# mkocabas/EpipolarPose

Measured on AMD Instinct MI355X. Metric: images/sec (4-view 256x256, ResNet-50) at 1/2/4/8 MI355X; MPJPE vs ref, higher is better.
Workload: dtype bf16; 1 GPU; configs[1]: ResNet-50 Integral-pose, 4-view 256x256 synthetic, batch=32/GPU, fully-supervised SmoothL1 loss; global_batch=32, joints=17, depth_res=64, optimizer=adam, parallelism=dp1, launch=eager, streams=2, deterministic=True

## Files before the change

### epipolarpose_amd/csrc/head_gemm.hip

```cpp
#include "common.h"
#include "bn_affine.h"
#include <algorithm>
#include <cstdlib>
#include <mutex>
#include <type_traits>
#include <unordered_map>
#include <utility>
#include <vector>

namespace epi {

typedef __bf16 bf16x8 __attribute__((ext_vector_type(8)));
typedef float f32x16 __attribute__((ext_vector_type(16)));

constexpr int GBK = 64;

template <int TM_, int WM_, int WN_, int MIN_WAVES_, int NSTAGE_, bool STAGGER_ = false> struct GemmCfg {
    static constexpr int TM = TM_, WM = WM_, WN = WN_, NW = WM_ * WN_, THREADS = 64 * NW, MIN_WAVES = MIN_WAVES_, NSTAGE = NSTAGE_;
    static constexpr bool STAGGER = STAGGER_;
    static constexpr int BM = WM_ * TM_ * 32, BN = WN_ * 64;
    static constexpr int A_BYTES = BM * 128, B_BYTES = BN * 128, STAGE_BYTES = A_BYTES + B_BYTES;
    static constexpr int AP = BM / 8 / NW, BP = BN / 8 / NW;
    static constexpr bool EARLY = NW == 4 && NSTAGE_ == 2;
    static_assert(AP >= 1 && BP >= 1 && BM % (8 * NW) == 0 && BN % (8 * NW) == 0, "whole pieces per wave");
// ... 1099 lines not shown
    if (OUT_F32) {
        *reinterpret_cast<float4v*>(reinterpret_cast<float*>(p.C) + orow * p.ldc + n) = a;
    } else {
        if (p.addend) {
            const uint2 r = *reinterpret_cast<const uint2*>(p.addend + orow * p.ldc + n);
            a.x = bf16_to_f32(f32_to_bf16(a.x)) + __uint_as_float(r.x << 16); a.y = bf16_to_f32(f32_to_bf16(a.y)) + __uint_as_float(r.x & 0xffff0000u);
            a.z = bf16_to_f32(f32_to_bf16(a.z)) + __uint_as_float(r.y << 16); a.w = bf16_to_f32(f32_to_bf16(a.w)) + __uint_as_float(r.y & 0xffff0000u);
        }
        uint2 o;
        o.x = pack_bf16x2(a.x, a.y);
        o.y = pack_bf16x2(a.z, a.w);
        *reinterpret_cast<uint2*>(reinterpret_cast<unsigned short*>(p.C) + orow * p.ldc + n) = o;
    }
}

constexpr int FS_ROWS = 32;
__global__ __launch_bounds__(256) void splitk_finish_stats_kernel(const float* __restrict__ slabs, int nsplit, GemmArgs p) {
    __shared__ float red[4][2][256];
    const int tx = threadIdx.x & 63, ty = threadIdx.x >> 6;
    const int col_tiles = (p.N + 255) / 256;
    const int tile_m = blockIdx.x / col_tiles, tile_n = blockIdx.x - tile_m * col_tiles;
    const int n = tile_n * 256 + tx * 4;
    float s1[4] = {0.f, 0.f, 0.f, 0.f}, s2[4] = {0.f, 0.f, 0.f, 0.f};
    if (n < p.N) {
        for (int r = ty; r < FS_ROWS; r += 4) {
            const int m = tile_m * FS_ROWS + r;
            if (m >= p.M) break;
            float4v a; a.x = a.y = a.z = a.w = 0.f;
            for (int sp = 0; sp < nsplit; ++sp) {
                const float4v v = *reinterpret_cast<const float4v*>(slabs + ((long long)sp * p.M + m) * p.N + n);
                a.x += v.x; a.y += v.y; a.z += v.z; a.w += v.w;
            }
            uint2 o;
            o.x = pack_bf16x2(a.x, a.y);
            o.y = pack_bf16x2(a.z, a.w);
            *reinterpret_cast<uint2*>(reinterpret_cast<unsigned short*>(p.C) + (long long)m * p.ldc + n) = o;
            const float v[4] = {__uint_as_float(o.x << 16), __uint_as_float(o.x & 0xffff0000u), __uint_as_float(o.y << 16), __uint_as_float(o.y & 0xffff0000u)};
#pragma unroll
            for (int e = 0; e < 4; ++e) { s1[e] += v[e]; s2[e] = fmaf(v[e], v[e], s2[e]); }
        }
    }
#pragma unroll
    for (int e = 0; e < 4; ++e) { red[ty][0][tx * 4 + e] = s1[e]; red[ty][1][tx * 4 + e] = s2[e]; }
    __syncthreads();
    float* dst = p.stats + (long long)(tile_m % p.stats_copies) * 2 * p.N;
    for (int t = threadIdx.x; t < 512; t += 256) {
        const int which = t >> 8, c = t & 255, col = tile_n * 256 + c;
        if (col < p.N) atomicAdd(dst + which * p.N + col, red[0][which][c] + red[1][which][c] + red[2][which][c] + red[3][which][c]);
    }
}

}

using namespace epi;

enum { CFG_SMALL = 0, CFG_TALL = 1, CFG_BIG = 2, CFG_HALF = 3, CFG_QUARTER = 4 };
struct GemmPlan { int cfg; int nsplit, kps; long long tiles; int pipe; };

static int g_tile_force_fwd();
static int gemm_tile_override() {
    const int v = 0;
    const int f = g_tile_force_fwd();
    return f == 1 || f == 2 ? f : (f == 5 ? 2 : v);
}

static int g_pipe_force_fwd();
static int gemm_pipe_mode() {
    const int v = 0;
    const int f = g_pipe_force_fwd();
    return f >= 0 ? f : v;
}

static int g_store_policy = -1;
static int gemm_store_policy() {
    if (g_store_policy < 0) g_store_policy = 0;
    return g_store_policy;
}
extern "C" int epi_gemm_store_policy(int v) {
    const int before = gemm_store_policy();
    if (v >= 0) g_store_policy = v;
    return before;
}
static int g_tile_force = 0, g_pipe_force = -1;
extern "C" int epi_gemm_tune(int tile, int pipe) {
    if (tile >= 0) g_tile_force = tile;
    if (pipe >= -1) g_pipe_force = pipe;
    return g_tile_force;
}

static int g_tile_force_fwd() { return g_tile_force; }
static int g_pipe_force_fwd() { return g_pipe_force; }

static GemmPlan gemm_plan_cfg(int cfg, int M, int N, int K, int nphase, bool pipe = false) {
    GemmPlan pl;
    pl.cfg = cfg;
    pl.pipe = pipe ? 1 : 0;
    const int bm = cfg == CFG_SMALL ? 128 : (cfg == CFG_HALF || cfg == CFG_QUARTER ? 64 : 256);
    const int bn = cfg == CFG_BIG ? 256 : (cfg == CFG_TALL || cfg == CFG_QUARTER ? 64 : 128);
    pl.tiles = (long long)((M + bm - 1) / bm) * ((N + bn - 1) / bn);
    const long long wgs = pl.tiles * nphase;
    const bool one_per_cu = cfg == CFG_BIG || pipe;
    const long long enough_env = 120;
    const long long enough = enough_env, target = one_per_cu ? 256 : 512;
    int nsplit = 1;
    if (wgs < enough) {
        nsplit = (int)(target / wgs);
// ... 114 lines not shown
}
extern "C" int epi_conv3x3_patch_mode(int mode) {
    const int before = patch_mode();
    if (mode >= 0 && mode <= 2) g_patch_mode = mode;
    return before;
}
static PatchPlan patch_plan(int M, int N, int Cs, int W, size_t workspace_bytes) {
    PatchPlan pl = {};
    const int nchunks = Cs / GBK;
    pl.cfg = N <= 64 ? PATCH_NARROW : PATCH_WIDE;
    if (pl.cfg == PATCH_WIDE && (long long)((M + 255) / 256) * ((N + 127) / 128) < 200) pl.cfg = PATCH_HALF;
    const int bm = pl.cfg == PATCH_HALF ? 128 : 256, bn = pl.cfg == PATCH_NARROW ? 64 : 128;
    const int tm = pl.cfg == PATCH_WIDE ? 2 : 1, wmv = pl.cfg == PATCH_NARROW ? 8 : 4;
    pl.patch_px = (bm + 2 * W + 2 + 7) / 8 * 8;
    if (pl.patch_px > 8 * 8 * PATCH_APW) return pl;
    const size_t epi = (size_t)8 * tm * 32 * 128 + (size_t)wmv * 2 * bn * sizeof(float);
    pl.single = pl.cfg == PATCH_NARROW && nchunks == 1;
    for (pl.nb = 3; pl.nb >= 2; --pl.nb) {
        pl.lds = std::max((size_t)(pl.single ? 1 : 2) * pl.patch_px * 128 + (size_t)pl.nb * bn * 128 + 1024 + 128, epi);
        if (pl.lds <= 160 * 1024) break;
    }
    if (pl.nb < 2) return pl;
    pl.tiles = (long long)((M + bm - 1) / bm) * ((N + bn - 1) / bn);
    pl.nsplit = 1;
    if (pl.tiles < 120) {
        if (patch_mode() < 2) return pl;
        pl.nsplit = (int)std::min<long long>(nchunks, std::max<long long>(1, 256 / pl.tiles));
    }
    while (pl.nsplit > 1 && (size_t)pl.nsplit * M * N * sizeof(float) > workspace_bytes) --pl.nsplit;
    pl.cps = (nchunks + pl.nsplit - 1) / pl.nsplit;
    pl.nsplit = (nchunks + pl.cps - 1) / pl.cps;
    pl.ok = pl.tiles <= 0x7fffffffLL;
    return pl;
}
static bool patch_eligible(const GemmArgs& a, bool out_f32, int nphase) {
    if (patch_mode() == 0 || out_f32 || nphase != 1 || !a.ga.enabled || a.ph.enabled || a.sc.enabled || a.bias || !a.coalesce) return false;
    if (a.ga.stride != 1 || a.ga.Hg != a.ga.Hs || a.ga.Wg != a.ga.Ws || a.ga.Cs % GBK || a.K != PATCH_TAPS * a.ga.Cs || a.ga.pitch) return false;
    for (int t = 0; t < PATCH_TAPS; ++t)
        if (a.ga.dy[t] < -1 || a.ga.dy[t] > 1 || a.ga.dx[t] < -1 || a.ga.dx[t] > 1) return false;
    return (long long)a.M * a.ga.Cs < (1LL << 31) && gemm_tile_override() == 0;
}
template <typename Cfg, int NB, bool SINGLE = false, bool RED = false>
static int launch_patch_red(const GemmArgs& a, const PatchPlan& pl, hipStream_t st) {
    static const hipError_t attr = hipFuncSetAttribute(reinterpret_cast<const void*>(&conv_patch_kernel<Cfg, NB, SINGLE, RED>),
                                                       hipFuncAttributeMaxDynamicSharedMemorySize, 160 * 1024);
    if (attr != hipSuccess) return EPI_ERR_LAUNCH;
    hipLaunchKernelGGL((conv_patch_kernel<Cfg, NB, SINGLE, RED>), dim3((unsigned)pl.tiles, (unsigned)pl.nsplit), dim3(Cfg::THREADS), pl.lds, st, a);
    EPI_CHECK_LAUNCH();
    return EPI_OK;
}
template <typename Cfg, int NB, bool SINGLE = false>
static int launch_patch(const GemmArgs& a, const PatchPlan& pl, hipStream_t st) {
    return a.br.z ? launch_patch_red<Cfg, NB, SINGLE, true>(a, pl, st) : launch_patch_red<Cfg, NB, SINGLE, false>(a, pl, st);
}

static int launch_gemm(GemmArgs a, bool out_f32, int nphase, void* workspace, size_t workspace_bytes, hipStream_t st, int* stats_done = nullptr,
                       int* red_done = nullptr) {
    if (stats_done) *stats_done = 0;
    if (red_done) *red_done = 0;
    a.store_policy = gemm_store_policy();
    const bool fuse_red = true;
    GemmBnRed want_red = a.br;
    a.br = GemmBnRed{};
    const long long red_max_rows = 1LL << 40;
    const long long red_min_rows = 0;
    if (deterministic() || !fuse_red || !red_done || !want_red.z || !want_red.bn || !want_red.sums || a.stats || a.bias ||
        ((reinterpret_cast<uintptr_t>(want_red.z) | reinterpret_cast<uintptr_t>(want_red.y)) & 15u) || (long long)a.M * nphase > red_max_rows ||
        (long long)a.M * nphase < red_min_rows)
        want_red.z = nullptr;
    if (a.addend && (out_f32 || (reinterpret_cast<uintptr_t>(a.addend) & 15u))) return EPI_ERR_UNSUPPORTED;
    a.coalesce = (!out_f32 && a.N % 8 == 0 && a.ldc % 8 == 0) ? 1 : 0;
    const bool half_addend = a.addend && a.addend_step == 2;
    if (half_addend && (!a.coalesce || a.ga.enabled || a.sc.enabled || a.ph.enabled || nphase != 1 || a.add_h <= 0 || a.add_w <= 0 || ((a.add_h | a.add_w) & 1) ||
                        (long long)a.M % ((long long)a.add_h * a.add_w)))
        return EPI_ERR_UNSUPPORTED;
    const bool fuse_stats = true;
    float* const want_stats = (fuse_stats && !deterministic()) ? a.stats : nullptr;
    a.stats = nullptr;
    if (!a.A || !a.Bt || !a.C || a.M <= 0 || a.N <= 0 || a.K <= 0) return EPI_ERR_INVALID_ARGUMENT;
    if (a.K % 8 || a.ldb % 8 || a.ldc % 4 || (!a.ga.enabled && a.lda % 8)) return EPI_ERR_UNSUPPORTED;
    if ((reinterpret_cast<uintptr_t>(a.A) | reinterpret_cast<uintptr_t>(a.Bt) | reinterpret_cast<uintptr_t>(a.C)) & 15u) return EPI_ERR_UNSUPPORTED;
    if (a.ga.enabled && (a.ga.Cs % GBK)) return EPI_ERR_UNSUPPORTED;
    if (a.bn_in_on) {
        if (out_f32 || a.ga.enabled || a.sc.enabled || a.ph.enabled || nphase != 1 || a.K % GBK || a.K > 2048 || want_red.z || a.bias || a.addend || !a.coalesce ||
            !a.bn_in.gamma || !a.bn_in.beta || !a.bn_in.scale || !a.bn_in.shift)
            return EPI_ERR_UNSUPPORTED;
        const GemmPlan pl = gemm_plan_cfg(CFG_SMALL, a.M, a.N, a.K, 1);
        if (pl.tiles > 0x7fffffffLL) return EPI_ERR_UNSUPPORTED;
        if (pl.nsplit > 1) {
            if (!workspace || (size_t)pl.nsplit * a.M * a.N * sizeof(float) > workspace_bytes) return EPI_ERR_WORKSPACE;
            a.slabs = (float*)workspace;
        }
        a.k_per_split = pl.kps;
        if (want_stats && pl.nsplit == 1) { a.stats = want_stats; if (stats_done) *stats_done = 1; }
        const int rc = launch_gemm_mode<false, CfgSmall, A_PLAIN, false, true>(a, pl, 1, st);
        if (rc != EPI_OK) return rc;
        if (pl.nsplit > 1) {
            if (want_stats && a.N % 4 == 0) {
                a.stats = want_stats;
                if (stats_done) *stats_done = 1;
                const unsigned blocks = (unsigned)(((a.M + FS_ROWS - 1) / FS_ROWS) * ((a.N + 255) / 256));
                hipLaunchKernelGGL(splitk_finish_stats_kernel, dim3(blocks), dim3(256), 0, st, a.slabs, pl.nsplit, a);
            } else {
                const long long n = (long long)a.M * (a.N >> 2);
                hipLaunchKernelGGL(splitk_finish_kernel<false>, dim3((unsigned)((n + 255) / 256)), dim3(256), 0, st, a.slabs, pl.nsplit, 1, a);
            }
            EPI_CHECK_LAUNCH();
        }
        return EPI_OK;
    }
    const bool stats_off_astat = true;
    if (!want_red.z && !(want_stats && stats_off_astat && !a.bias) && !half_addend &&
        !out_f32 && !a.ga.enabled && !a.sc.enabled && nphase == 1 && (a.K == 64 || a.K == 128 || a.K == 256) && a.N % 8 == 0 &&
        a.ldc % 8 == 0 && a.N >= 4 * AS_BN && a.N <= 8192 && a.M >= 64 * AS_BM && gemm_tile_override() == 0) {
        const unsigned grid = (unsigned)((a.M + AS_BM - 1) / AS_BM);
        const bool astat_stats = false;
        if (want_stats && !a.bias && astat_stats) { a.stats = want_stats; if (stats_done) *stats_done = 1; }
#define EPI_ASTAT(KS)                                                                                                      \
        do {                                                                                                               \
            const size_t lds = AS_RING * (size_t)AS_BN * 32 * KS + AS_WAVES * 4096 + (size_t)((a.N + AS_BN - 1) / AS_BN) * AS_BN * 4 * 3;                                          \
            static const hipError_t attr = hipFuncSetAttribute(reinterpret_cast<const void*>(&head_gemm_astat_kernel<KS>),  \
                                                               hipFuncAttributeMaxDynamicSharedMemorySize, (int)lds);      \
            if (attr != hipSuccess) return EPI_ERR_LAUNCH;                                                                 \
            hipLaunchKernelGGL((head_gemm_astat_kernel<KS>), dim3(grid), dim3(AS_THREADS), lds, st, a);                     \
        } while (0)
        if (a.K == 256) EPI_ASTAT(16);
        else if (a.K == 128) EPI_ASTAT(8);
        else EPI_ASTAT(4);
#undef EPI_ASTAT
        EPI_CHECK_LAUNCH();
        return EPI_OK;
    }
    if (patch_eligible(a, out_f32, nphase)) {
        const PatchPlan pp = patch_plan(a.M, a.N, a.ga.Cs, a.ga.Wg, workspace ? workspace_bytes : 0);
        if (pp.ok) {
            a.patch_px = pp.patch_px;
            a.chunks_per_split = pp.cps;
            if (pp.nsplit > 1) a.slabs = (float*)workspace;
            else if (want_stats) { a.stats = want_stats; if (stats_done) *stats_done = 1; }
            else if (want_red.z) { a.br = want_red; *red_done = 1; }
            int rc;
            if (pp.cfg == PATCH_NARROW && pp.single) rc = pp.nb == 3 ? launch_patch<PatchNarrow, 3, true>(a, pp, st) : launch_patch<PatchNarrow, 2, true>(a, pp, st);
            else if (pp.cfg == PATCH_NARROW) rc = pp.nb == 3 ? launch_patch<PatchNarrow, 3>(a, pp, st) : launch_patch<PatchNarrow, 2>(a, pp, st);
            else if (pp.cfg == PATCH_HALF) rc = pp.nb == 3 ? launch_patch<PatchHalf, 3>(a, pp, st) : launch_patch<PatchHalf, 2>(a, pp, st);
            else rc = pp.nb == 3 ? launch_patch<PatchWide, 3>(a, pp, st) : launch_patch<PatchWide, 2>(a, pp, st);
            if (rc != EPI_OK) return rc;
            if (pp.nsplit > 1) {
                if (want_stats && !a.addend) {
                    a.stats = want_stats;
                    if (stats_done) *stats_done = 1;
                    const unsigned blocks = (unsigned)(((a.M + FS_ROWS - 1) / FS_ROWS) * ((a.N + 255) / 256));
                    hipLaunchKernelGGL(splitk_finish_stats_kernel, dim3(blocks), dim3(256), 0, st, a.slabs, pp.nsplit, a);
                } else {
                    const long long n = (long long)a.M * (a.N >> 2);
                    hipLaunchKernelGGL(splitk_finish_kernel<false>, dim3((unsigned)((n + 255) / 256)), dim3(256), 0, st, a.slabs, pp.nsplit, 1, a);
                }
                EPI_CHECK_LAUNCH();
            }
            return EPI_OK;
        }
    }
    GemmPlan pl = gemm_plan(a.M, a.N, a.K, a.ldc, nphase, out_f32);
    if (want_red.z && pl.pipe && pl.cfg != CFG_SMALL) pl = gemm_plan(a.M, a.N, a.K, a.ldc, nphase, out_f32, false);
    if (pl.tiles > 0x7fffffffLL) return EPI_ERR_UNSUPPORTED;
    if (half_addend && pl.nsplit > 1) return EPI_ERR_UNSUPPORTED;
    if (pl.nsplit > 1) {
        if (!workspace || (size_t)pl.nsplit * nphase * a.M * a.N * sizeof(float) > workspace_bytes) return EPI_ERR_WORKSPACE;
        a.slabs = (float*)workspace;
    }
    a.k_per_split = pl.kps;
    if (want_stats && pl.nsplit == 1 && a.coalesce && !a.bias) { a.stats = want_stats; if (stats_done) *stats_done = 1; }
    if (want_red.z && pl.nsplit == 1 && a.coalesce && (!pl.pipe || pl.cfg == CFG_SMALL) && (pl.cfg == CFG_BIG || pl.cfg == CFG_SMALL || pl.cfg == CFG_TALL)) {
        a.br = want_red;
        *red_done = 1;
    }
    int rc;
    if (a.br.z) rc = pl.cfg == CFG_BIG ? launch_gemm_cfg<false, CfgBig, true>(a, pl, nphase, st)
                   : (pl.cfg == CFG_TALL ? launch_gemm_cfg<false, CfgTall, true>(a, pl, nphase, st)
                      : (pl.pipe ? launch_gemm_cfg<false, CfgSmallP, true>(a, pl, nphase, st) : launch_gemm_cfg<false, CfgSmall, true>(a, pl, nphase, st)));
    else if (pl.cfg == CFG_BIG) rc = g_tile_force == 5 ? launch_gemm_cfg<false, CfgBigLock>(a, pl, nphase, st) : launch_gemm_cfg<false, CfgBig>(a, pl, nphase, st);
    else if (out_f32) rc = launch_gemm_cfg<true, CfgSmall>(a, pl, nphase, st);
    else if (pl.cfg == CFG_HALF) rc = launch_gemm_cfg<false, CfgHalf>(a, pl, nphase, st);
    else if (pl.cfg == CFG_QUARTER) rc = launch_gemm_cfg<false, CfgQuarter>(a, pl, nphase, st);
    else if (pl.cfg == CFG_TALL) rc = pl.pipe ? launch_gemm_cfg<false, CfgTallP>(a, pl, nphase, st) : launch_gemm_cfg<false, CfgTall>(a, pl, nphase, st);
// ... 1267 lines not shown
```

### epipolarpose_amd/hip.py

```python
import ctypes
import os

import torch

_LIB_DIR = os.environ.get("EPI_LIB_DIR") or os.path.join(os.path.dirname(os.path.abspath(__file__)), "_lib")
_LIB_PATH = os.path.join(_LIB_DIR, "libepipolar_hip.so")
_lib = None

EPI_F32, EPI_BF16, EPI_F64 = 0, 1, 2
EPI_NCHW, EPI_NHWC = 0, 1
LOSS_KINDS = {"l1": 0, "l2": 1, "smoothl1": 2}
TRI_METHODS = {"iterative": 0, "ls": 1, "dlt": 2, "poly": 3}

_vp, _i, _d, _sz = ctypes.c_void_p, ctypes.c_int, ctypes.c_double, ctypes.c_size_t


class EpiViewMeta(ctypes.Structure):
    _fields_ = [(k, _vp) for k in ("center_x", "center_y", "width", "height", "scale", "rot", "R", "T", "f", "c", "P")]


_SIGNATURES = {
    "epi_version": (ctypes.c_char_p, []),
    "epi_status_string": (ctypes.c_char_p, [_i]),
    "epi_softargmax3d_workspace_bytes": (_sz, [_i] * 5),
    "epi_softargmax3d_fwd": (_i, [_vp, _i, _i, _i, _i, _i, _i, _i, _vp, _vp, _vp, _vp, _sz, _vp]),
    "epi_softargmax3d_bwd": (_i, [_vp, _i, _i, _i, _i, _i, _i, _i, _vp, _vp, _vp, _vp, _vp, _vp, _vp]),
    "epi_softargmax3d_bwd_colsums": (_i, [_vp, _i, _i, _i, _i, _i, _i, _i, _vp, _vp, _vp, _vp, _vp, _vp, _vp, ctypes.POINTER(ctypes.c_int), _vp]),
    "epi_joint_loss": (_i, [_vp, _vp, _vp, _i, _i, _i, _i, _i, _vp, _vp, _vp]),
    "epi_argmax_workspace_bytes": (_sz, [_i, _i]),
    "epi_argmax_rows": (_i, [_vp, _i, _i, _i, _vp, _vp, _vp, _sz, _vp]),
    "epi_decode_to_image": (_i, [_vp, _i, _i, ctypes.POINTER(EpiViewMeta), _d, _d, _d, _vp, _vp]),
    "epi_triangulate_iterls": (_i, [_vp, _i, _vp, _i, _i, _i, _i, _d, _i, _vp, _vp, _vp]),
    "epi_triangulate_ls": (_i, [_vp, _i, _vp, _i, _i, _i, _i, _vp, _vp, _vp]),
    "epi_triangulate_dlt": (_i, [_vp, _i, _vp, _i, _i, _i, _i, _vp, _vp, _vp]),
    "epi_triangulate_poly": (_i, [_vp, _i, _vp, _i, _i, _i, _i, _vp, _vp, _vp]),
    "epi_triangulate_staged": (_i, [_i]),
    "epi_fundamental_8point": (_i, [_vp, _vp, _i, _i, _vp, _vp, _vp]),
    "epi_fundamental_lmeds_medians": (_i, [_vp, _i, _vp, _vp, _i, _vp, _vp]),
    "epi_fundamental_errors": (_i, [_vp, _vp, _vp, _i, _vp, _vp]),
    "epi_correct_matches": (_i, [_vp, _vp, _vp, _i, _i, _vp, _vp, _vp]),
    "epi_reproject_labels": (_i, [_vp, _i, _i, _i, ctypes.POINTER(EpiViewMeta), _d, _d, _d, _i, _vp, _vp, _vp]),
    "epi_self_supervision": (_i, [_vp, _i, _i, _i, ctypes.POINTER(EpiViewMeta), _d, _d, _d, _i, _i, _d, _i, _vp, _vp, _vp, _vp]),
    "epi_gemm_workspace_bytes": (_sz, [_i, _i, _i, _i]),
    "epi_gemm_bf16": (_i, [_vp, _i, _vp, _i, _vp, _i, _i, _i, _i, _i, _vp, _vp, _sz, _vp]),
    "epi_deconv4x4s2_pack_weight": (_i, [_vp, _i, _i, _vp, _vp, _vp]),
    "epi_deconv4x4s2_fwd": (_i, [_vp, _vp, _vp, _i, _i, _i, _i, _i, _vp, _sz, _vp]),
    "epi_deconv4x4s2_fwd_stats": (_i, [_vp, _vp, _vp, _i, _i, _i, _i, _i, _vp, _vp, _vp, _sz, _vp]),
    "epi_deconv4x4s2_bwd_data": (_i, [_vp, _vp, _vp, _i, _i, _i, _i, _i, _vp, _sz, _vp]),
    "epi_conv2d_workspace_bytes": (_sz, [_i] * 9),
    "epi_conv2d_fwd": (_i, [_vp, _vp, _vp, _i, _i, _i, _i, _i, _i, _i, _i, _i, _vp, _vp, _vp, _sz, _vp]),
    "epi_conv1x1_fwd_bn_in": (_i, [_vp, _vp, _i, ctypes.c_float, ctypes.c_float, _vp, _vp, _i, _i, _i, _i, _i, _vp, _vp, _vp, _sz, _vp]),
    "epi_conv2d_pack_weight_bwd": (_i, [_vp, _i, _i, _i, _i, _i, _i, _vp, _vp]),
    "epi_conv2d_pack_row_bytes": (_sz, []),
    "epi_conv2d_pack_fill_row": (_i, [_vp, _vp, _vp, _i, _i, _i, _i, _i, _i, ctypes.c_longlong, ctypes.POINTER(ctypes.c_longlong)]),
    "epi_conv2d_pack_weight_bwd_multi": (_i, [_vp, _i, ctypes.c_longlong, _vp]),
    "epi_conv2d_bwd_data": (_i, [_vp, _vp, _vp, _i, _i, _i, _i, _i, _i, _i, _i, _i, _vp, _vp, _sz, _vp]),
    "epi_conv2d_bwd_data_bnred": (_i, [_vp, _vp, _vp, _i, _i, _i, _i, _i, _i, _i, _i, _i, _vp, _i, _vp, _vp, _vp, _sz, _vp]),
    "epi_conv2d_bwd_data_half_addend_ok": (_i, [_i, _i, _i, _i, _i]),
    "epi_deconv4x4s2_bwd_data_bnred": (_i, [_vp, _vp, _vp, _i, _i, _i, _i, _i, _vp, _vp, _vp, _sz, _vp]),
    "epi_gemm_bf16_bnred": (_i, [_vp, _i, _vp, _i, _vp, _i, _i, _i, _i, _vp, _vp, _vp, _sz, _vp]),
    "epi_bn_finalize": (_i, [_vp, ctypes.c_longlong, _i, ctypes.c_float, ctypes.c_float, _i, _vp]),
    "epi_maxpool3x3s2_bn_relu_fwd": (_i, [_vp, _vp, _vp, _vp, _i, _i, _i, _i, _vp]),
    "epi_bn_act_fwd_dual": (_i, [_vp, _vp, ctypes.c_longlong, _i, _vp, _vp, ctypes.c_float, ctypes.c_float, _i, _vp, _vp]),
    "epi_bn_act_bwd_reduced": (_i, [_vp, _vp, ctypes.c_longlong, _i, _vp, _vp, _vp, _vp, _vp, _vp, _vp, _vp, _vp]),
    "epi_conv2d_bwd_weight": (_i, [_vp, _vp, _vp, _i, _i, _i, _i, _i, _i, _i, _i, _i, _i, _vp, ctypes.c_size_t, _vp]),
    "epi_conv2d_bwd_weight_deferred": (_i, [_vp, _vp, _vp, _i, _i, _i, _i, _i, _i, _i, _i, _i, _i, _vp, ctypes.c_size_t, _vp, _vp]),
    "epi_slab_reduce_chunks": (ctypes.c_longlong, [ctypes.c_longlong]),
    "epi_slab_reduce_multi": (_i, [_vp, _i, ctypes.c_longlong, _vp]),
    "epi_wgrad_group_max": (_i, []),
    "epi_wgrad_group_plan": (_i, [_vp, _i, ctypes.POINTER(ctypes.c_size_t), ctypes.POINTER(ctypes.c_int)]),
    "epi_wgrad_group": (_i, [_vp, _i, _vp, _sz, _vp, _vp]),
    "epi_wgrad_item": (_i, [_vp, _vp, _sz, _vp, _vp]),
    "epi_bn_sum_copies": (_i, [_i]),
    "epi_conv3x3_patch_mode": (_i, [_i]),
    "epi_gemm_tune": (_i, [_i, _i]),
    "epi_gemm_store_policy": (_i, [_i]),
    "epi_set_deterministic": (_i, [_i]),
    "epi_bn_act_fwd": (_i, [_vp, _vp, ctypes.c_longlong, _i, _vp, _vp, ctypes.c_float, ctypes.c_float, _i, _i, _vp, _vp, _vp, _vp,
                            _vp, _vp, _vp, _vp, _vp, _vp]),
    "epi_bn_act_bwd": (_i, [_vp, _vp, _vp, ctypes.c_longlong, _i, _vp, _vp, _vp, _vp, _i, _vp, _vp, _vp, _vp, _vp, _vp]),
    "epi_gemm_tn_workspace_bytes": (_sz, [_i, _i, _i, _i]),
    "epi_gemm_tn_plan": (_i, [_i, _i, _i, _i, ctypes.POINTER(ctypes.c_longlong)]),
    "epi_gemm_tn_bf16": (_i, [_vp, _i, _vp, _i, _vp, _i, _i, _i, _vp, _sz, _vp]),
    "epi_deconv4x4s2_bwd_weight": (_i, [_vp, _vp, _vp, _i, _i, _i, _i, _i, _i, _vp, _sz, _vp]),
    "epi_deconv4x4s2_pack_phase_cl": (_i, [_vp, _i, _i, _vp, _vp]),
    "epi_deconv4x4s2_pack_fill_row": (_i, [_vp, _vp, _vp, _i, _i, ctypes.c_longlong, ctypes.POINTER(ctypes.c_longlong)]),
    "epi_column_sums_bf16": (_i, [_vp, ctypes.c_longlong, _i, _vp, _vp]),
    "epi_stem7x7s2_s2d_bytes": (_sz, [_i, _i, _i]),
    "epi_stem7x7s2_workspace_bytes": (_sz, [_i, _i, _i, _i]),
    "epi_stem7x7s2_s2d": (_i, [_vp, _i, _i, _i, _i, _i, _vp, _vp]),
    "epi_stem7x7s2_pack_weight": (_i, [_vp, _i, _i, _vp, _vp]),
    "epi_stem7x7s2_unpack_weight_grad": (_i, [_vp, _i, _i, _vp, _i, _vp]),
    "epi_stem7x7s2_fwd": (_i, [_vp, _vp, _vp, _i, _i, _i, _i, _vp, _vp, _vp, _sz, _vp]),
    "epi_stem7x7s2_bwd_weight": (_i, [_vp, _vp, _vp, _i, _i, _i, _i, _vp, _sz, _vp]),
    "epi_split_bf16": (_i, [_vp, ctypes.c_longlong, _i, _vp, _i, _i, _vp, _vp]),
    "epi_conv2d_fwd_f32": (_i, [_vp, _vp, _vp, _i, _i, _i, _i, _i, _i, _i, _i, _i, _vp, _sz, _vp]),
    "epi_conv2d_bwd_data_f32": (_i, [_vp, _vp, _vp, _i, _i, _i, _i, _i, _i, _i, _i, _i, _vp, _sz, _vp]),
    "epi_deconv4x4s2_fwd_f32": (_i, [_vp, _vp, _vp, _i, _i, _i, _i, _i, _vp, _sz, _vp]),
    "epi_deconv4x4s2_bwd_data_f32": (_i, [_vp, _vp, _vp, _i, _i, _i, _i, _i, _vp, _sz, _vp]),
    "epi_bn_act_fwd_f32": (_i, [_vp, _vp, ctypes.c_longlong, _i, _vp, _vp, ctypes.c_float, ctypes.c_float, _i, _i, _vp, _vp, _vp, _vp,
                                _vp, _vp, _vp, _vp, _vp, _vp]),
    "epi_bn_act_bwd_f32": (_i, [_vp, _vp, _vp, ctypes.c_longlong, _i, _vp, _vp, _vp, _vp, _i, _vp, _vp, _vp, _vp, _vp, _vp]),
    "epi_column_sums_f32": (_i, [_vp, ctypes.c_longlong, _i, _vp, _vp]),
    "epi_maxpool3x3s2_fwd_f32": (_i, [_vp, _vp, _vp, _i, _i, _i, _i, _vp]),
    "epi_maxpool3x3s2_bwd_f32": (_i, [_vp, _vp, _vp, _i, _i, _i, _i, _vp]),
    "epi_adam_tensor_bytes": (_sz, []),
    "epi_adam_chunk_elems": (_i, []),
    "epi_adam_step": (_i, [_vp, _vp, _i, ctypes.c_float, ctypes.c_float, ctypes.c_float, ctypes.c_float, ctypes.c_longlong, _vp]),
    "epi_adam_step_clipped": (_i, [_vp, _vp, _i, ctypes.c_float, ctypes.c_float, ctypes.c_float, ctypes.c_float, ctypes.c_longlong,
                                   ctypes.c_float, _vp, _vp]),
    "epi_dropout_bf16": (_i, [_vp, _vp, ctypes.c_longlong, ctypes.c_float, ctypes.c_ulonglong, _vp]),
    "epi_maxpool3x3s2_fwd": (_i, [_vp, _vp, _vp, _i, _i, _i, _i, _vp]),
    "epi_maxpool3x3s2_bwd": (_i, [_vp, _vp, _vp, _i, _i, _i, _i, _vp]),
    "epi_crop_patches": (_i, [_vp, _vp, _vp, _vp, _vp, _vp, ctypes.POINTER(ctypes.c_float), ctypes.POINTER(ctypes.c_float), _i, _i, _i, _vp,
                              _i, _i, _vp]),
    "epi_crop_patches_occluded": (_i, [_vp, _vp, _vp, _vp, _vp, _vp, ctypes.POINTER(ctypes.c_float), ctypes.POINTER(ctypes.c_float), _i, _i, _i, _vp,
                                       _vp, _vp, _vp, _i, _vp, _i, _i, _vp]),
    "epi_evaluate_poses": (_i, [_vp, _vp, _vp, _vp, _vp, _i, _i, _i, _vp, _i, _vp, _vp, _vp]),
}
EXPORTED_SYMBOLS = tuple(_SIGNATURES)


def lib_path():
    return _LIB_PATH


class _Library:

    def __init__(self, cdll, path, missing):
# ... 867 lines not shown
```

### include/epipolar_hip.h

```cpp
#ifndef EPIPOLAR_HIP_H
#define EPIPOLAR_HIP_H

#include <stddef.h>
#include <stdint.h>

#ifdef __cplusplus
extern "C" {
#endif

typedef void* epi_stream_t;

enum epi_status {
    EPI_OK = 0,
    EPI_ERR_INVALID_ARGUMENT = 1,
    EPI_ERR_UNSUPPORTED = 2,
    EPI_ERR_WORKSPACE = 3,
    EPI_ERR_LAUNCH = 4
};

enum epi_dtype { EPI_F32 = 0, EPI_BF16 = 1, EPI_F64 = 2 };
enum epi_layout {
    EPI_NCHW = 0,
    EPI_NHWC = 1
};
// ... 89 lines not shown

int epi_deconv4x4s2_bwd_data(const void* dy, const void* w_bwd, void* dx, int B, int H, int W, int Cin, int Cout,
                             void* workspace, size_t workspace_bytes, epi_stream_t stream);

int epi_bn_sum_copies(int C);
int epi_bn_act_fwd(const void* x, const void* residual, long long R, int C, const float* gamma, const float* beta,
                   float eps, float momentum, int training, int relu, float* running_mean, float* running_var,
                   long long* num_batches_tracked, float* mean, float* rstd, float* scale_shift, float* sums_ws,
                   float* bwd_sums, void* y, epi_stream_t stream);
int epi_bn_act_bwd(const void* dy, const void* x, const void* y, long long R, int C, const float* gamma,
                   const float* mean, const float* rstd, const float* scale_shift, int relu,
                   float* dbeta_dgamma, void* dx, void* dres, float* fwd_sums_clear, float* param_grads, epi_stream_t stream);

typedef struct EpiBnLayer {
    const float* gamma;
    const float* beta;
    float* running_mean;
    float* running_var;
    long long* num_batches_tracked;
    float* mean;
    float* rstd;
    float* scale_shift;
    float* sums_ws;
    float* bwd_sums;
} EpiBnLayer;
int epi_bn_act_fwd_dual(const void* x, const void* x_proj, long long R, int C, const EpiBnLayer* main_bn, const EpiBnLayer* proj_bn,
                        float eps, float momentum, int training, void* y, epi_stream_t stream);
int epi_bn_finalize(const EpiBnLayer* layer, long long R, int C, float eps, float momentum, int training, epi_stream_t stream);
int epi_maxpool3x3s2_bn_relu_fwd(const void* x, const float* scale_shift, void* y, void* pos, int B, int H, int W, int C, epi_stream_t stream);

typedef struct EpiBnReduce {
    const void* z;
    const void* y;
    const float* bn;
    float* sums;
    int relu;
} EpiBnReduce;
int epi_bn_act_bwd_reduced(const void* dz, const void* x, long long R, int C, const float* gamma, const float* mean, const float* rstd,
                           const float* scale_shift, const float* dbeta_dgamma, void* dx, float* fwd_sums_clear, float* param_grads,
                           epi_stream_t stream);
int epi_conv2d_bwd_data_bnred(const void* dy, const void* w_bwd, void* dx, int B, int H, int W, int Cin, int Cout, int KH, int KW,
                              int stride, int pad, const void* addend, int addend_step, const EpiBnReduce* red, int* red_done, void* workspace,
                              size_t workspace_bytes, epi_stream_t stream);
int epi_conv2d_bwd_data_half_addend_ok(int B, int H, int W, int Cin, int Cout);
int epi_deconv4x4s2_bwd_data_bnred(const void* dy, const void* w_bwd, void* dx, int B, int H, int W, int Cin, int Cout,
                                   const EpiBnReduce* red, int* red_done, void* workspace, size_t workspace_bytes, epi_stream_t stream);
int epi_gemm_bf16_bnred(const void* A, int lda, const void* Bt, int ldb, void* C, int ldc, int M, int N, int K, const EpiBnReduce* red,
                        int* red_done, void* workspace, size_t workspace_bytes, epi_stream_t stream);

size_t epi_conv2d_workspace_bytes(int B, int H, int W, int Cin, int Cout, int KH, int KW, int stride, int pad);
int epi_conv3x3_patch_mode(int mode);
int epi_gemm_tune(int tile, int pipe);
int epi_gemm_store_policy(int policy);
int epi_conv2d_fwd(const void* x, const void* w, void* y, int B, int H, int W, int Cin, int Cout, int KH, int KW,
                   int stride, int pad, float* bn_sums, int* bn_sums_done, void* workspace, size_t workspace_bytes,
                   epi_stream_t stream);
int epi_conv1x1_fwd_bn_in(const void* z, const EpiBnLayer* in_bn, int in_training, float eps, float momentum, const void* w, void* y, int B, int H, int W,
                          int Cin, int Cout, float* bn_sums, int* bn_sums_done, void* workspace, size_t workspace_bytes, epi_stream_t stream);
int epi_conv2d_pack_weight_bwd(const void* w, int Cout, int Cin, int KH, int KW, int stride, int pad, void* w_bwd,
                               epi_stream_t stream);
size_t epi_conv2d_pack_row_bytes(void);
int epi_conv2d_pack_fill_row(void* row_host, const void* w, void* w_bwd, int Cout, int Cin, int KH, int KW, int stride, int pad,
                             long long tile_begin, long long* ntiles);
int epi_conv2d_pack_weight_bwd_multi(const void* rows, int nrows, long long total_tiles, epi_stream_t stream);
int epi_conv2d_bwd_data(const void* dy, const void* w_bwd, void* dx, int B, int H, int W, int Cin, int Cout, int KH, int KW,
                        int stride, int pad, const void* addend, void* workspace, size_t workspace_bytes, epi_stream_t stream);

int epi_conv2d_bwd_weight(const void* x, const void* dy, void* dw, int dw_dtype, int B, int H, int W, int Cin, int Cout,
                          int KH, int KW, int stride, int pad, void* workspace, size_t workspace_bytes, epi_stream_t stream);
typedef struct EpiSlabReduce {
    const float* slabs;
    void* out;
    long long n;
    long long chunk_begin;
    int nsplit, out_bf16;
} EpiSlabReduce;
int epi_conv2d_bwd_weight_deferred(const void* x, const void* dy, void* dw, int dw_dtype, int B, int H, int W, int Cin, int Cout,
                                   int KH, int KW, int stride, int pad, void* workspace, size_t workspace_bytes,
                                   EpiSlabReduce* pending, epi_stream_t stream);
long long epi_slab_reduce_chunks(long long n);
int epi_slab_reduce_multi(const EpiSlabReduce* rows_dev, int nrows, long long total_chunks, epi_stream_t stream);

enum { EPI_WGRAD_CONV2D = 0, EPI_WGRAD_DECONV4X4S2 = 1 };
typedef struct EpiWgradItem {
    const void* x;
    const void* dy;
    void* dw;
    int dw_dtype, kind;
    int B, H, W, Cin, Cout, KH, KW, stride, pad;
    const float* x_scale_shift;
} EpiWgradItem;
int epi_wgrad_group_max(void);
int epi_wgrad_group_plan(const EpiWgradItem* items, int n, size_t* slab_bytes, int* nsplit);
int epi_wgrad_group(const EpiWgradItem* items, int n, void* slab_ws, size_t slab_bytes, EpiSlabReduce* pending, epi_stream_t stream);
int epi_wgrad_item(const EpiWgradItem* item, void* workspace, size_t workspace_bytes, EpiSlabReduce* pending, epi_stream_t stream);

size_t epi_gemm_tn_workspace_bytes(int R, int I, int J, int ntap);
int epi_gemm_tn_plan(int R, int I, int J, int ntap, long long* plan);
int epi_gemm_tn_bf16(const void* A, int lda, const void* B, int ldb, float* C, int R, int I, int J,
                     void* workspace, size_t workspace_bytes, epi_stream_t stream);
int epi_deconv4x4s2_bwd_weight(const void* x, const void* dy, void* dw_taps, int dw_dtype, int B, int H, int W, int Cin, int Cout,
                               void* workspace, size_t workspace_bytes, epi_stream_t stream);
int epi_column_sums_bf16(const void* x, long long R, int C, float* sums, epi_stream_t stream);

size_t epi_adam_tensor_bytes(void);
int epi_adam_chunk_elems(void);
// ... 57 lines not shown
```

Before: 5258 images/s.

## Add weight-resident streaming GEMM kernel for skinny-K 1x1 convs with fused stats

Adds a new streaming GEMM kernel for GEMMs with K of 64, 128 or 256. Each workgroup keeps a column block of the weights in LDS and walks a contiguous range of row blocks, double-buffering A fragments in registers. It can fuse the BN column-sum statistics, an addend, and the BN-reduce epilogue. By default it is used only for large-M cases (fused reduction, or stats with K=64), replacing the general tiled path there. The goal is to cut repeated weight loads and per-tile overhead on these memory-bound 1x1 convolutions, in exchange for a larger launch surface and atomic stat accumulation across row ranges.

```diff
diff --git a/epipolarpose_amd/csrc/head_gemm.hip b/epipolarpose_amd/csrc/head_gemm.hip
--- a/epipolarpose_amd/csrc/head_gemm.hip
+++ b/epipolarpose_amd/csrc/head_gemm.hip
@@ -1175,6 +1175,8 @@
 
 }
 
+#include "stream_gemm.h"
+
 using namespace epi;
 
 enum { CFG_SMALL = 0, CFG_TALL = 1, CFG_BIG = 2, CFG_HALF = 3, CFG_QUARTER = 4 };
@@ -1395,6 +1397,90 @@
 template <typename Cfg, int NB, bool SINGLE = false>
 static int launch_patch(const GemmArgs& a, const PatchPlan& pl, hipStream_t st) {
     return a.br.z ? launch_patch_red<Cfg, NB, SINGLE, true>(a, pl, st) : launch_patch_red<Cfg, NB, SINGLE, false>(a, pl, st);
+}
+
+static int g_stream_mode = -1, g_stream_max_wg = 0;
+static int stream_mode() {
+    if (g_stream_mode < 0) {
+        const char* e = getenv("EPI_GEMM_STREAM");
+        g_stream_mode = (e && e[0] >= '0' && e[0] <= '2' && !e[1]) ? e[0] - '0' : 1;
+    }
+    return g_stream_mode;
+}
+extern "C" int epi_gemm_stream(int mode, int max_workgroups) {
+    const int before = stream_mode();
+    if (mode >= 0) {
+        if (mode > 2) return before;
+        g_stream_mode = mode;
+        g_stream_max_wg = max_workgroups > 0 ? max_workgroups : 0;
+    }
+    return before;
+}
+enum { STREAM_SUMS = 1, STREAM_RED = 2, STREAM_ADDEND = 4, STREAM_HALF_ADDEND = 8, STREAM_BIAS = 16, STREAM_F32 = 32, STREAM_INDEXED = 64, STREAM_FLAGS = 127 };
+static int stream_bn(int N, int K, int flags) {
+    const int cap = (flags & STREAM_RED) ? 64 : std::min((flags & STREAM_SUMS) ? 128 : 256, 32768 / (2 * K));
+    for (int bn = cap; bn >= 64; bn >>= 1)
+        if (N % bn == 0) return bn;
+    return 0;
+}
+static int stream_eligible(int M, int N, int K, int lda, int ldb, int ldc, int flags) {
+    if (flags & (STREAM_HALF_ADDEND | STREAM_BIAS | STREAM_F32 | STREAM_INDEXED)) return 0;
+    if ((flags & STREAM_SUMS) && (flags & (STREAM_ADDEND | STREAM_RED))) return 0;
+    if (K != 64 && K != 128 && K != 256) return 0;
+    if (N % 64 || N > 8192 || lda % 8 || ldb % 8 || ldc % 8 || lda < K || ldb < K || ldc < N) return 0;
+    if (!stream_bn(N, K, flags)) return 0;
+    if ((long long)M * std::max(lda, ldc) * 2 >= (1LL << 31)) return 0;
+    const bool planned = M >= 32768 && ((flags & STREAM_RED) || ((flags & STREAM_SUMS) && K == 64));
+    return planned ? 3 : 1;
+}
+extern "C" int epi_gemm_stream_eligible(int M, int N, int K, int flags) {
+    if (M <= 0 || N <= 0 || K <= 0 || flags < 0 || (flags & ~STREAM_FLAGS)) return -EPI_ERR_INVALID_ARGUMENT;
+    return stream_eligible(M, N, K, K, K, N, flags);
+}
+
+template <int KS, int BN, int MODE, bool ADD, int MASK>
+static int launch_stream_inst(const StreamArgs& s, unsigned grid, hipStream_t st) {
+    constexpr size_t lds = StreamCfg<KS, BN>::LDS;
+    hipLaunchKernelGGL((stream_gemm_kernel<KS, BN, MODE, ADD, MASK>), dim3(grid), dim3(ST_THREADS), lds, st, s);
+    EPI_CHECK_LAUNCH();
+    return EPI_OK;
+}
+template <int KS, int BN>
+static int launch_stream_kb(const StreamArgs& s, int mode, bool add, int mask, unsigned grid, hipStream_t st) {
+    if (mode == ST_RED) {
+        if constexpr (BN == 64) {
+            if (mask == ST_MASK_Y) return add ? launch_stream_inst<KS, BN, ST_RED, true, ST_MASK_Y>(s, grid, st) : launch_stream_inst<KS, BN, ST_RED, false, ST_MASK_Y>(s, grid, st);
+            if (mask == ST_MASK_Z) return add ? launch_stream_inst<KS, BN, ST_RED, true, ST_MASK_Z>(s, grid, st) : launch_stream_inst<KS, BN, ST_RED, false, ST_MASK_Z>(s, grid, st);
+            return add ? launch_stream_inst<KS, BN, ST_RED, true, ST_MASK_NONE>(s, grid, st) : launch_stream_inst<KS, BN, ST_RED, false, ST_MASK_NONE>(s, grid, st);
+        } else {
+            return EPI_ERR_UNSUPPORTED;
+        }
+    }
+    if (mode == ST_STATS) {
+        if constexpr (BN <= 128) return launch_stream_inst<KS, BN, ST_STATS, false, ST_MASK_NONE>(s, grid, st);
+        else return EPI_ERR_UNSUPPORTED;
+    }
+    return add ? launch_stream_inst<KS, BN, ST_PLAIN, true, ST_MASK_NONE>(s, grid, st) : launch_stream_inst<KS, BN, ST_PLAIN, false, ST_MASK_NONE>(s, grid, st);
+}
+static int launch_stream(const GemmArgs& a, int flags, hipStream_t st) {
+    StreamArgs s = {};
+    s.A = a.A; s.Bt = a.Bt; s.C = reinterpret_cast<unsigned short*>(a.C); s.addend = a.addend; s.stats = a.stats;
+    s.M = a.M; s.N = a.N; s.lda = a.lda; s.ldb = a.ldb; s.ldc = a.ldc; s.stats_copies = a.stats_copies > 0 ? a.stats_copies : 1;
+    s.row_blocks = (a.M + ST_BM - 1) / ST_BM;
+    s.br = a.br;
+    const int bn = stream_bn(a.N, a.K, flags), nb = a.N / bn;
+    int ranges = std::min(std::max(1, (nb == 1 ? 256 : 512) / nb), std::max(1, s.row_blocks / 2));
+    if (g_stream_max_wg > 0) ranges = std::min(ranges, std::max(1, g_stream_max_wg / nb));
+    const int per = (s.row_blocks + ranges - 1) / ranges;
+    ranges = (s.row_blocks + per - 1) / per;
+    const unsigned grid = (unsigned)(nb * ranges);
+    const int mode = a.br.z ? ST_RED : (a.stats ? ST_STATS : ST_PLAIN);
+    const int mask = !a.br.relu ? ST_MASK_NONE : (a.br.y ? ST_MASK_Y : ST_MASK_Z);
+    const bool add = a.addend != nullptr;
+    if (a.K == 64) return bn == 256 ? launch_stream_kb<4, 256>(s, mode, add, mask, grid, st)
+                          : (bn == 128 ? launch_stream_kb<4, 128>(s, mode, add, mask, grid, st) : launch_stream_kb<4, 64>(s, mode, add, mask, grid, st));
+    if (a.K == 128) return bn == 128 ? launch_stream_kb<8, 128>(s, mode, add, mask, grid, st) : launch_stream_kb<8, 64>(s, mode, add, mask, grid, st);
+    return launch_stream_kb<16, 64>(s, mode, add, mask, grid, st);
 }
 
 static int launch_gemm(GemmArgs a, bool out_f32, int nphase, void* workspace, size_t workspace_bytes, hipStream_t st, int* stats_done = nullptr,
@@ -1452,10 +1538,17 @@
         }
         return EPI_OK;
     }
+    int stream_flags = 0, stream_take = 0;
+    {
+        stream_flags = (want_stats ? STREAM_SUMS : 0) | (want_red.z ? STREAM_RED : 0) | (a.addend ? (half_addend ? STREAM_HALF_ADDEND : STREAM_ADDEND) : 0) |
+                       (a.bias ? STREAM_BIAS : 0) | (out_f32 ? STREAM_F32 : 0) | ((a.ga.enabled || a.sc.enabled || a.ph.enabled || nphase != 1) ? STREAM_INDEXED : 0);
+        const int el = g_tile_force == 0 && stream_mode() > 0 ? stream_eligible(a.M, a.N, a.K, a.lda, a.ldb, a.ldc, stream_flags) : 0;
+        stream_take = stream_mode() == 2 ? (el & 1) : (el & 2);
+    }
     const bool stats_off_astat = true;
     if (!want_red.z && !(want_stats && stats_off_astat && !a.bias) && !half_addend &&
         !out_f32 && !a.ga.enabled && !a.sc.enabled && nphase == 1 && (a.K == 64 || a.K == 128 || a.K == 256) && a.N % 8 == 0 &&
-        a.ldc % 8 == 0 && a.N >= 4 * AS_BN && a.N <= 8192 && a.M >= 64 * AS_BM && gemm_tile_override() == 0) {
+        a.ldc % 8 == 0 && a.N >= 4 * AS_BN && a.N <= 8192 && a.M >= 64 * AS_BM && gemm_tile_override() == 0 && !(stream_take && stream_mode() == 2)) {
         const unsigned grid = (unsigned)((a.M + AS_BM - 1) / AS_BM);
         const bool astat_stats = false;
         if (want_stats && !a.bias && astat_stats) { a.stats = want_stats; if (stats_done) *stats_done = 1; }
@@ -1473,6 +1566,11 @@
 #undef EPI_ASTAT
         EPI_CHECK_LAUNCH();
         return EPI_OK;
+    }
+    if (stream_take) {
+        if (want_stats) { a.stats = want_stats; if (stats_done) *stats_done = 1; }
+        if (want_red.z) { a.br = want_red; *red_done = 1; }
+        return launch_stream(a, stream_flags, st);
     }
     if (patch_eligible(a, out_f32, nphase)) {
         const PatchPlan pp = patch_plan(a.M, a.N, a.ga.Cs, a.ga.Wg, workspace ? workspace_bytes : 0);
diff --git a/epipolarpose_amd/csrc/stream_gemm.h b/epipolarpose_amd/csrc/stream_gemm.h
--- /dev/null
+++ b/epipolarpose_amd/csrc/stream_gemm.h
@@ -0,0 +1,202 @@
+#pragma once
+
+namespace epi {
+
+enum { ST_PLAIN = 0, ST_STATS = 1, ST_RED = 2 };
+enum { ST_MASK_NONE = 0, ST_MASK_Z = 1, ST_MASK_Y = 2 };
+constexpr int ST_THREADS = 256, ST_BM = 128, ST_PARK = 4 * 4096;
+
+template <int KSTEPS, int BN> struct StreamCfg {
+    static constexpr int K = 16 * KSTEPS, PITCH = 2 * K + 16, W_BYTES = BN * PITCH, NJ = BN / 64;
+    static constexpr int COLS = W_BYTES + ST_PARK;
+    static constexpr int LDS = W_BYTES + ST_PARK + (BN == 64 ? 4 * BN * 4 : 0);
+    static_assert(BN % 64 == 0 && BN <= 256 && BN * K * 2 <= 32768, "weight block of at most 32 KiB");
+    static_assert(3 * LDS <= 160 * 1024, "three workgroups per CU");
+    static_assert(2 * BN * sizeof(float) <= 4096, "the waves' column-sum rows fit their park slices");
+};
+
+struct StreamArgs {
+    const unsigned short* A;
+    const unsigned short* Bt;
+    unsigned short* C;
+    const unsigned short* addend;
+    float* stats;
+    int M, N, lda, ldb, ldc, stats_copies;
+    int row_blocks;
+    GemmBnRed br;
+};
+
+template <int KSTEPS, int BN, int MODE, bool ADD, int MASK>
+__global__ __launch_bounds__(ST_THREADS, 3) void stream_gemm_kernel(StreamArgs p) {
+    typedef StreamCfg<KSTEPS, BN> Cfg;
+    constexpr int K = Cfg::K, PITCH = Cfg::PITCH, NJ = Cfg::NJ;
+    constexpr bool SUMS = MODE != ST_PLAIN, RED = MODE == ST_RED;
+    static_assert(!RED || BN == 64, "fused reduction: 64-column blocks");
+    constexpr bool TWO_SETS = MODE == ST_PLAIN ? KSTEPS <= 8 : (MODE == ST_STATS && KSTEPS <= 4);
+    constexpr bool A_AT_TOP = RED && KSTEPS == 16;
+    constexpr bool PRE_EARLY = KSTEPS <= 8;
+    constexpr bool AD_EARLY = PRE_EARLY && !(RED && KSTEPS == 8);
+    constexpr bool Y_EARLY = PRE_EARLY && !(KSTEPS == 8 && ADD);
+    extern __shared__ __attribute__((aligned(16))) char smem[];
+    const int tid = threadIdx.x, lane = tid & 63, wid = tid >> 6;
+    const int frow = lane & 31, fhalf = lane >> 5, c8 = lane & 7, r8 = lane >> 3;
+    const int nb = p.N / BN, ranges = (int)gridDim.x / nb;
+    const int lid = xcd_remap(blockIdx.x, gridDim.x);
+    const int cb = lid % nb, g = lid / nb;
+    const int n0 = cb * BN;
+    const int b_begin = (int)((long long)g * p.row_blocks / ranges), b_end = (int)((long long)(g + 1) * p.row_blocks / ranges);
+
+    auto load_a = [&](int blk, uint4v (&f)[KSTEPS]) __attribute__((always_inline)) {
+        const int m = min(blk * ST_BM + wid * 32 + frow, p.M - 1);
+        const unsigned boff = ((unsigned)m * (unsigned)p.lda + 8u * fhalf) * 2u;
+        const uint4v* arow = reinterpret_cast<const uint4v*>(reinterpret_cast<const char*>(p.A) + boff);
+#pragma unroll
+        for (int ks = 0; ks < KSTEPS; ++ks) f[ks] = arow[2 * ks];
+    };
+    uint4v af[KSTEPS], afn[TWO_SETS ? KSTEPS : 1];
+    if (!A_AT_TOP && b_begin < b_end) load_a(b_begin, af);
+    {
+        constexpr int CPR = K / 8;
+        for (int c = tid; c < BN * CPR; c += ST_THREADS) {
+            const int r = c / CPR, ch = c - r * CPR;
+            *reinterpret_cast<uint4v*>(smem + r * PITCH + ch * 16) = *reinterpret_cast<const uint4v*>(p.Bt + (long long)(n0 + r) * p.ldb + ch * 8);
+        }
+    }
+    float* cols_s = reinterpret_cast<float*>(smem + Cfg::COLS);
+    if (RED)
+        for (int c = tid; c < 4 * BN; c += ST_THREADS) cols_s[c] = p.br.bn[(c / BN) * p.N + n0 + (c % BN)];
+    __syncthreads();
+    const char* wfrag = smem + frow * PITCH + fhalf * 16;
+    char* mine = smem + Cfg::W_BYTES + wid * 4096;
+
+    GemmBnRed br = p.br;
+    br.relu = MASK != ST_MASK_NONE ? 1 : 0;
+    if (MASK != ST_MASK_Y) br.y = nullptr;
+    float ssum[SUMS ? NJ : 1][8], ssq[SUMS ? NJ : 1][8];
+#pragma unroll
+    for (int j = 0; j < (SUMS ? NJ : 1); ++j)
+#pragma unroll
+        for (int k = 0; k < 8; ++k) { ssum[j][k] = 0.f; ssq[j][k] = 0.f; }
+    br.bn = nullptr;
+
+    for (int blk = b_begin; blk < b_end; ++blk) {
+        if constexpr (TWO_SETS) { if (blk + 1 < b_end) load_a(blk + 1, afn); }
+        if (A_AT_TOP) load_a(blk, af);
+        const int m_first = blk * ST_BM + wid * 32 + r8;
+#pragma unroll
+        for (int j = 0; j < NJ; ++j) {
+            const int n = n0 + j * 64 + c8 * 8;
+            uint4v ad[ADD ? 4 : 1], zpre[RED ? 4 : 1], ypre[(RED && MASK == ST_MASK_Y) ? 4 : 1];
+            auto prefetch = [&](bool want_ad, bool want_zy, bool want_y) __attribute__((always_inline)) {
+                if (!((ADD && want_ad) || (RED && (want_zy || want_y)))) return;
+#pragma unroll
+                for (int it = 0; it < 4; ++it) {
+                    const int m = m_first + 8 * it;
+                    const unsigned boff = ((unsigned)min(m, p.M - 1) * (unsigned)p.ldc + (unsigned)n) * 2u;
+                    if (ADD && want_ad) ad[it] = *reinterpret_cast<const uint4v*>(reinterpret_cast<const char*>(p.addend) + boff);
+                    if (RED && want_zy) zpre[it] = *reinterpret_cast<const uint4v*>(reinterpret_cast<const char*>(br.z) + boff);
+                    if (RED && want_y && MASK == ST_MASK_Y) ypre[it] = *reinterpret_cast<const uint4v*>(reinterpret_cast<const char*>(br.y) + boff);
+                }
+            };
+            prefetch(AD_EARLY, PRE_EARLY, Y_EARLY);
+            f32x16 acc[2];
+#pragma unroll
+            for (int t = 0; t < 2; ++t)
+#pragma unroll
+                for (int r = 0; r < 16; ++r) acc[t][r] = 0.f;
+            uint4v fb[2][2];
+            auto read_b = [&](int ks, uint4v (&f)[2]) __attribute__((always_inline)) {
+#pragma unroll
+                for (int tj = 0; tj < 2; ++tj) f[tj] = *reinterpret_cast<const uint4v*>(wfrag + (j * 64 + tj * 32) * PITCH + ks * 32);
+            };
+            read_b(0, fb[0]);
+#pragma unroll
+            for (int ks = 0; ks < KSTEPS; ++ks) {
+                if (ks + 1 < KSTEPS) read_b(ks + 1, fb[(ks + 1) & 1]);
+                __builtin_amdgcn_sched_barrier(0);
+#pragma unroll
+                for (int tj = 0; tj < 2; ++tj)
+                    acc[tj] = __builtin_amdgcn_mfma_f32_32x32x16_bf16(__builtin_bit_cast(bf16x8, fb[ks & 1][tj]), __builtin_bit_cast(bf16x8, af[ks]), acc[tj], 0, 0, 0);
+            }
+            if constexpr (!TWO_SETS && !A_AT_TOP) if (j == NJ - 1) {
+                __builtin_amdgcn_sched_barrier(0);
+                if (blk + 1 < b_end) load_a(blk + 1, af);
+                __builtin_amdgcn_sched_barrier(0);
+            }
+            prefetch(!AD_EARLY, !PRE_EARLY, !Y_EARLY);
+#pragma unroll
+            for (int tj = 0; tj < 2; ++tj)
+#pragma unroll
+                for (int q = 0; q < 4; ++q) {
+                    uint2 t;
+                    t.x = pack_bf16x2(acc[tj][4 * q], acc[tj][4 * q + 1]);
+                    t.y = pack_bf16x2(acc[tj][4 * q + 2], acc[tj][4 * q + 3]);
+                    const int unit = tj * 8 + 2 * q + fhalf;
+                    *reinterpret_cast<uint2*>(mine + frow * 128 + ((unit ^ (frow & 15)) << 3)) = t;
+                }
+            BnRedCols rcols;
+            if (RED) {
+                const float* cs = cols_s + j * 64 + c8 * 8;
+#pragma unroll
+                for (int k = 0; k < 8; ++k) { rcols.mu[k] = cs[k]; rcols.rs[k] = cs[BN + k]; rcols.sc[k] = cs[2 * BN + k]; rcols.sh[k] = cs[3 * BN + k]; }
+            }
+            const int SJ = SUMS ? j : 0;
+#pragma unroll
+            for (int it = 0; it < 4; ++it) {
+                const int row = it * 8 + r8, sw = row & 15;
+                const uint2 lo = *reinterpret_cast<const uint2*>(mine + row * 128 + (((2 * c8) ^ sw) << 3));
+                const uint2 hi = *reinterpret_cast<const uint2*>(mine + row * 128 + (((2 * c8 + 1) ^ sw) << 3));
+                const int m = m_first + 8 * it;
+                if (m >= p.M) continue;
+                if (MODE == ST_STATS) {
+                    const unsigned int w4[4] = {lo.x, lo.y, hi.x, hi.y};
+#pragma unroll
+                    for (int k = 0; k < 4; ++k) {
+                        const float a = __uint_as_float(w4[k] << 16), b = __uint_as_float(w4[k] & 0xffff0000u);
+                        ssum[SJ][2 * k] += a; ssq[SJ][2 * k] = fmaf(a, a, ssq[SJ][2 * k]);
+                        ssum[SJ][2 * k + 1] += b; ssq[SJ][2 * k + 1] = fmaf(b, b, ssq[SJ][2 * k + 1]);
+                    }
+                }
+                uint4v o; o.x = lo.x; o.y = lo.y; o.z = hi.x; o.w = hi.y;
+                if (ADD) o = add_bf16x8(o, ad[it]);
+                if (RED) o = bnred_apply(br, o, zpre[it], MASK == ST_MASK_Y ? ypre[it] : uint4v{0u, 0u, 0u, 0u}, rcols, ssum[SJ], ssq[SJ]);
+                *reinterpret_cast<uint4v*>(reinterpret_cast<char*>(p.C) + ((unsigned)m * (unsigned)p.ldc + (unsigned)n) * 2u) = o;
+            }
+        }
+        if constexpr (TWO_SETS) {
+#pragma unroll
+            for (int ks = 0; ks < KSTEPS; ++ks) af[ks] = afn[ks];
+        }
+    }
+    if (SUMS) {
+#pragma unroll
+        for (int j = 0; j < NJ; ++j)
+#pragma unroll
+            for (int k = 0; k < 8; ++k) {
+#pragma unroll
+                for (int o = 8; o < 64; o <<= 1) { ssum[j][k] += __shfl_xor(ssum[j][k], o, 64); ssq[j][k] += __shfl_xor(ssq[j][k], o, 64); }
+            }
+        float* st = reinterpret_cast<float*>(smem + Cfg::W_BYTES);
+        if (lane < 8) {
+#pragma unroll
+            for (int j = 0; j < NJ; ++j) {
+                float* row = st + wid * 1024 + j * 64 + c8 * 8;
+                *reinterpret_cast<float4v*>(row) = float4v{ssum[j][0], ssum[j][1], ssum[j][2], ssum[j][3]};
+                *reinterpret_cast<float4v*>(row + 4) = float4v{ssum[j][4], ssum[j][5], ssum[j][6], ssum[j][7]};
+                *reinterpret_cast<float4v*>(row + BN) = float4v{ssq[j][0], ssq[j][1], ssq[j][2], ssq[j][3]};
+                *reinterpret_cast<float4v*>(row + BN + 4) = float4v{ssq[j][4], ssq[j][5], ssq[j][6], ssq[j][7]};
+            }
+        }
+        __syncthreads();
+        float* dst = RED ? br.sums : p.stats + (long long)(g % p.stats_copies) * 2 * p.N;
+        for (int t = tid; t < 2 * BN; t += ST_THREADS) {
+            float v = 0.f;
+#pragma unroll
+            for (int w = 0; w < 4; ++w) v += st[w * 1024 + t];
+            const int which = t / BN, col = n0 + (t - which * BN);
+            atomicAdd(dst + which * p.N + col, v);
+        }
+    }
+}
+
+}
diff --git a/epipolarpose_amd/hip.py b/epipolarpose_amd/hip.py
--- a/epipolarpose_amd/hip.py
+++ b/epipolarpose_amd/hip.py
@@ -75,6 +75,8 @@
     "epi_conv3x3_patch_mode": (_i, [_i]),
     "epi_gemm_tune": (_i, [_i, _i]),
     "epi_gemm_store_policy": (_i, [_i]),
+    "epi_gemm_stream": (_i, [_i, _i]),
+    "epi_gemm_stream_eligible": (_i, [_i, _i, _i, _i]),
     "epi_set_deterministic": (_i, [_i]),
     "epi_bn_act_fwd": (_i, [_vp, _vp, ctypes.c_longlong, _i, _vp, _vp, ctypes.c_float, ctypes.c_float, _i, _i, _vp, _vp, _vp, _vp,
                             _vp, _vp, _vp, _vp, _vp, _vp]),
diff --git a/include/epipolar_hip.h b/include/epipolar_hip.h
--- a/include/epipolar_hip.h
+++ b/include/epipolar_hip.h
@@ -165,6 +165,8 @@
 int epi_conv3x3_patch_mode(int mode);
 int epi_gemm_tune(int tile, int pipe);
 int epi_gemm_store_policy(int policy);
+int epi_gemm_stream(int mode, int max_workgroups);
+int epi_gemm_stream_eligible(int M, int N, int K, int flags);
 int epi_conv2d_fwd(const void* x, const void* w, void* y, int B, int H, int W, int Cin, int Cout, int KH, int KW,
                    int stride, int pad, float* bn_sums, int* bn_sums_done, void* workspace, size_t workspace_bytes,
                    epi_stream_t stream);
```

Result: no change. 5311 images/s (median of 6 runs) (+1.0%).
